# src-d/kmcuda

Measured on AMD Instinct MI355X. Metric: point-assignments/sec per Lloyd iter (8Mx256@1024), higher is better.
Workload: dtype f32

## Files before the change

kmcuda_amd/csrc/engine.cpp:

```cpp
#include "engine.hpp"

#include <math.h>
#include <stdio.h>
#include <stdlib.h>
#include <string.h>

#include <mutex>
#include <vector>

#include "../../include/kmcuda_amd.h"

namespace kmx {

int g_verbosity = 0;

namespace {
std::mutex g_stream_pool_mutex;
std::vector<std::vector<hipStream_t>> g_stream_pool;
}

hipStream_t pooled_stream_acquire(int device) {
  {
    std::lock_guard<std::mutex> lock(g_stream_pool_mutex);
    if ((size_t)device < g_stream_pool.size() && !g_stream_pool[device].empty()) {
// ... 68 lines not shown
  for (auto &s : spans_) { (void)hipEventDestroy(s.a); (void)hipEventDestroy(s.b); }
  for (void *p : owned_) (void)hipFree(p);
  if (pinned_) (void)hipHostFree(pinned_);
  if (side_stream_ && own_side_stream_) pooled_stream_release(device_, side_stream_);
  if (ev_fork_) (void)hipEventDestroy(ev_fork_);
  if (ev_join_) (void)hipEventDestroy(ev_join_);
  for (hipEvent_t e : ev_report_)
    if (e) (void)hipEventDestroy(e);
  if (ev_rows_) (void)hipEventDestroy(ev_rows_);
  if (own_stream_ && stream_) {
    if (blocking_stream_) (void)hipStreamDestroy(stream_);
    else pooled_stream_release(device_, stream_);
  }
}

int Engine::init(int device, uint32_t n_rows, uint32_t D, uint32_t K, int metric, int fp16x2, hipStream_t stream) {
  if (getenv("KMCUDA_AMD_DEBUG")) g_verbosity = atoi(getenv("KMCUDA_AMD_DEBUG"));
  if (const char *f = getenv("KMCUDA_AMD_FILTER")) filter_mode_ = strcmp(f, "f32") == 0 ? 1 : 0;
  if (const char *c = getenv("KMCUDA_AMD_ROW_CACHE")) row_cache_allowed_ = atoi(c) != 0;
  carry_pairs_ = true;
  if (const char *c = getenv("KMCUDA_AMD_CARRY_PAIRS")) carry_pairs_ = atoi(c) != 0;
  if (const char *c = getenv("KMCUDA_AMD_SETTLE")) settle_ = atoi(c) != 0;
  if (const char *c = getenv("KMCUDA_AMD_DUO")) { duo_on_ = atoi(c) != 0; duo_always_ = atoi(c) == 2; }
  if (const char *c = getenv("KMCUDA_AMD_WIDE")) wide_ok_ = atoi(c) != 0;
  if (const char *c = getenv("KMCUDA_AMD_GEMM")) wide_ok_ = atoi(c) != 0;
  if (const char *u = getenv("KMCUDA_AMD_UPDATE"))
    ms_.force = strcmp(u, "radix") == 0 ? 1 : (strcmp(u, "sync") == 0 ? 2 : (strcmp(u, "bucket") == 0 ? 3 : 0));
  if (D == 0 || K < 1 || K >= 0x7FFFFFFFu) return kInvalidArguments;
  if (fp16x2) return kInvalidArguments;
  int ndev = 0;
  if (hipGetDeviceCount(&ndev) != hipSuccess || device < 0 || device >= ndev) return kNoSuchDevice;
  KMX_HIP(hipSetDevice(device), kNoSuchDevice);
  device_ = device;
  if (stream == (hipStream_t)(intptr_t)-1) {
    KMX_HIP(hipStreamCreateWithFlags(&stream_, hipStreamDefault), kRuntimeError);
    own_stream_ = true;
    blocking_stream_ = true;
  } else if (stream) {
    stream_ = stream;
  } else {
    stream_ = pooled_stream_acquire(device);
    if (!stream_) return kRuntimeError;
    own_stream_ = true;
  }
  N_ = n_rows; D_ = D; K_ = K; metric_ = metric; fp16x2_ = fp16x2;
  K_pad_ = (K + 31) / 32 * 32;
// ... 341 lines not shown
    KMX_HIP(launch_centroid_rows(metric_, centroids, K_, D_, Kt_, csqr_, ct_, side_stream_), kRuntimeError);
    KMX_HIP(hipEventRecord(ev_rows_, side_stream_), kRuntimeError);
    rows_on_side = true;
    if (!prepared) {
      uint32_t *next = stats_;
      stats_ = stats_ == stats_base_ ? stats_base_ + 8 : stats_base_;
      KMX_HIP(launch_centroid_prep_frozen(metric_, centroids, K_, D_, K_pad_, DP_ ? DP_ : wide_dp_, mu_, finite_, bias_,
                                          bias2_, cfil_, panelhi_, stats_, next, counters_ + 1, counters_ + 3, counters_ + 4,
                                          carry_on_ ? drift_ : nullptr, carry_on_ && drift_ ? counters_ + kCarryCursor : nullptr,
                                          stream_),
              kRuntimeError);
      carry_preps_++;
    }
  } else {
    int rc = prepare_centroids(centroids);
    if (rc) return rc;
  }
  LloydArgs a;
  a.samples = samples; a.N = N_; a.D = D_; a.K = K_; a.K_pad = K_pad_; a.DP = DP_; a.Kt = Kt_;
  a.cfil = cfil_; a.bias = bias_; a.mu = mu_; a.ct = ct_; a.csqr = csqr_; a.stats = stats_;
  a.eps = eps_; a.tie_slack = tie_slack_;
  a.assignments = assignments; a.assignments_prev = assignments_prev;
  a.flagged = flagged_; a.pairs = pairs_; a.counters = counters_;
  if (N_ == 0) return kSuccess;
  if (wide_sel) {
    const int rc = lloyd_assign_wide(a, centroids, wide_steady, rows_on_side, carry_was_valid);
    if (rc != kNoSuchDevice + 100) return rc;
  }
  if (exact_only || DP_ == 0 || (DP_ > 256 && filter_mode_ != 0)) {
    span_begin(1);
    const uint32_t grid = N_ < 8192u ? N_ : 8192u;
    KMX_HIP(launch_lloyd_exact(metric_, a, nullptr, nullptr, grid, stream_), kRuntimeError);
    span_end();
    return kSuccess;
  }
  span_begin(0);
  if (two_stage) {
    const void *rows = half_rows_ ? half_rows_ : (const void *)samples;
    const bool half = half_rows_ != nullptr;
    bool duo_listed = false;
    if (!steady)
      KMX_HIP(launch_centroid_panelhi(centroids, K_, D_, K_pad_, DP_, finite_, mu_, bias_, panelhi_, stats_, stream_),
              kRuntimeError);
    if (build_cache) {
      const size_t npad = ((size_t)N_ + 255) / 256 * 256;
      if (!xcache_) {
// ... 615 lines not shown
```

kmcuda_amd/csrc/engine.hpp:

```cpp
#pragma once
#include <hip/hip_runtime.h>
#include <stdint.h>

#include <vector>

#include "kernels.hpp"

namespace kmx {

enum Result {
  kSuccess = 0, kInvalidArguments, kNoSuchDevice, kMemoryAllocationFailure, kRuntimeError, kMemoryCopyError
};

#define KMX_HIP(call, ret)                                                                   \
  do {                                                                                       \
    hipError_t e__ = (call);                                                                 \
    if (e__ != hipSuccess) {                                                                 \
      if (kmx::g_verbosity > 0)                                                              \
        printf("%s:%d -> %s (%s)\n", __FILE__, __LINE__, hipGetErrorString(e__), #call);     \
      return ret;                                                                            \
    }                                                                                        \
  } while (0)

extern int g_verbosity;
// ... 90 lines not shown

  int device_ = -1;
  hipStream_t stream_ = nullptr;
  bool own_stream_ = false, blocking_stream_ = false;
  hipStream_t side_stream_ = nullptr;
  bool own_side_stream_ = false;
  hipEvent_t ev_fork_ = nullptr, ev_join_ = nullptr;
  hipEvent_t ev_rows_ = nullptr;
  uint32_t N_ = 0, D_ = 0, K_ = 0, K_pad_ = 0, Kt_ = 0, DP_ = 0;
  int metric_ = 0, fp16x2_ = 0;
  bool strict_h2_ = false;
  float *h2_sq_ = nullptr;
  float eps_ = 0, tie_slack_ = 0;

  float *csqr_ = nullptr, *bias_ = nullptr, *bias2_ = nullptr, *cfil_ = nullptr, *ct_ = nullptr, *mu_ = nullptr;
  uint32_t *finite_ = nullptr;
  const void *half_rows_ = nullptr;
  void *panelhi_ = nullptr;
  uint32_t *undecided_ = nullptr;
  float *und_thr_ = nullptr;
  uint32_t *duo_ = nullptr;
  bool duo_on_ = true;
  bool duo_always_ = false;
  int filter_mode_ = 0;
  bool settle_ = true;
  uint32_t wide_dp_ = 0;
  bool wide_ok_ = true;
  bool wide_failed_ = false;
  void *wide_rows16_ = nullptr;
  float *wide_meta_ = nullptr;
  uint32_t *wide_cont_ = nullptr;
  int lloyd_assign_wide(const LloydArgs &a, const float *centroids, bool steady, bool rows_on_side, bool carry_was_valid);
  bool row_cache_allowed_ = true;
  bool row_cache_on_ = false, row_cache_valid_ = false, mu_frozen_ = false;
  void *xcache_ = nullptr;
  float *xmeta_ = nullptr;
  bool carry_on_ = false;
  bool carry_valid_ = false;
  uint32_t carry_preps_ = 0;
  uint32_t carry_seq_ = 0;
  CarryPolicy carry_policy_;
  float *ub_ = nullptr, *lb_ = nullptr, *drift_ = nullptr;
  bool carry_pairs_ = true;
  float *l3_ = nullptr;
  uint32_t *p1_ = nullptr, *p2_ = nullptr;
  uint32_t *carry_list_ = nullptr;
// ... 53 lines not shown
```

kmcuda_amd/csrc/kernels.hpp:

```cpp
#pragma once
#include <hip/hip_runtime.h>
#include <stdint.h>

namespace kmx {

struct LloydArgs {
  const float *samples;
  uint32_t N, D, K;
  uint32_t K_pad;
  uint32_t DP;
  uint32_t Kt;
  const float *cfil;
  const float *bias;
  const float *mu;
  const float *ct;
  const float *csqr;
  const uint32_t *stats;
  float eps;
  float tie_slack;
  uint32_t *assignments, *assignments_prev;
  uint32_t *flagged;
  uint32_t *pairs;
  uint32_t *counters;
};
constexpr uint32_t kWaveRowGridMax = 1u << 20;
inline uint32_t wave_row_grid(uint32_t n_rows) {
  const uint32_t g = (n_rows + 3u) / 4u;
  return g < kWaveRowGridMax ? (g ? g : 1u) : kWaveRowGridMax;
}
constexpr uint32_t kStopFlag = 8;
constexpr uint32_t kCarryCursor = 9, kCarrySkipped = 10;
constexpr uint32_t kCarryPaired = 12;
constexpr uint32_t kDuoCount = 14;
struct CarryArgs {
  float *ub = nullptr, *lb = nullptr;
  const uint32_t *row_list = nullptr;
  const uint32_t *n_list = nullptr;
  uint32_t *host_report = nullptr;
  uint32_t seq = 0;
  int angular = 0;
  float *l3 = nullptr;
  uint32_t *p1 = nullptr, *p2 = nullptr;
};
struct StopCtl {
  float threshold = -1.f;
  uint32_t *counters = nullptr;
// ... 295 lines not shown
```

kmcuda_amd/csrc/lloyd_carry.hip:

```cpp
#include <cstdlib>

#include "lloyd_coarse.hpp"
#include "lloyd_refine.hpp"

namespace kmx {

constexpr int kSkipRowsPerThread = 8, kSkipBlock = 256;
template <bool WIDE>
__global__ __launch_bounds__(kSkipBlock) void carry_skip_kernel(
    uint32_t N, uint32_t K, const uint32_t *__restrict__ assignments, uint32_t *__restrict__ assignments_prev,
    CarryArgs cy, const float2 *__restrict__ xmeta, const float *__restrict__ drift, const uint32_t *__restrict__ stats,
    float tie_slack, uint32_t *__restrict__ row_list, const uint32_t *__restrict__ finite, uint32_t *__restrict__ pairs,
    uint32_t *__restrict__ counters, int probe, float terms) {
  if (counters[kStopFlag] != 0u) return;
  float *__restrict__ ub = cy.ub, *__restrict__ lb = cy.lb, *__restrict__ l3 = cy.l3;
  const int angular = cy.angular;
  const float maxdrift = __uint_as_float(stats[6]);
  const float cmaxo = sqrtf(__uint_as_float(stats[2])) * 1.000001f;
  const float4 *__restrict__ wmeta = reinterpret_cast<const float4 *>(xmeta);
  const float mu_norm = WIDE ? wmeta[N].x : reinterpret_cast<const float *>(xmeta)[2 * (((size_t)N + 255) / 256 * 256)];
  const float u = 5.9604645e-8f;
  const float maxdb = __uint_as_float(stats[7]);
  const float cmaxc = sqrtf(__uint_as_float(stats[0])) * 1.000001f;
  const float eb = 4.0f * terms * u * mu_norm * (cmaxc + maxdrift);
// ... 114 lines not shown
                             float tie_slack, uint32_t *row_list, const uint32_t *finite, uint32_t *pairs,
                             uint32_t *counters, bool probe, hipStream_t st, uint32_t wide_dg) {
  const uint32_t chunk = kSkipBlock * kSkipRowsPerThread;
  if (wide_dg)
    hipLaunchKernelGGL(carry_skip_kernel<true>, dim3((N + chunk - 1) / chunk), dim3(kSkipBlock), 0, st, N, K, assignments,
                       assignments_prev, cy, reinterpret_cast<const float2 *>(xmeta), drift, stats, tie_slack, row_list,
                       finite, pairs, counters, probe ? 1 : 0, (float)(wide_dg + 8u));
  else
    hipLaunchKernelGGL(carry_skip_kernel<false>, dim3((N + chunk - 1) / chunk), dim3(kSkipBlock), 0, st, N, K, assignments,
                       assignments_prev, cy, reinterpret_cast<const float2 *>(xmeta), drift, stats, tie_slack, row_list,
                       finite, pairs, counters, probe ? 1 : 0, 520.0f);
  return hipGetLastError();
}

template <int DP>
static hipError_t launch_coarse_carry_dp(const LloydArgs &a, const void *rows, bool half_rows, const void *xcache,
                                         const float *xmeta, const void *panelhi, uint32_t *undecided, float *und_thr,
                                         const CarryArgs &cy, uint32_t rows_hint, uint32_t *duo, hipStream_t st) {
  constexpr int NSET = DP <= 256 ? 2 : 1;
  const size_t lds_bytes = 2 * 64 * (size_t)(DP * 2) + 512 + 64 + (size_t)DP * 4;
  const uint32_t rows_per_block = 128u * NSET;
  uint32_t grid = (a.N + rows_per_block - 1) / rows_per_block;
  const bool fast = a.D == (uint32_t)DP;
#define KMX_CARRY_LAUNCH(H, F, C, MODE, SRC)                                                                          \
  hipLaunchKernelGGL((lloyd_coarse2_kernel<DP, H, F, C, NSET, MODE>), dim3(grid), dim3(256), lds_bytes, st, SRC,      \
                     xmeta, a.N, a.D, reinterpret_cast<const float *>(panelhi), a.bias, a.mu, a.K_pad, a.K, a.stats,   \
                     a.eps, a.tie_slack, a.assignments, a.assignments_prev, undecided, und_thr, a.counters, cy, duo)
  if (!cy.row_list) {
    KMX_CARRY_LAUNCH(false, true, true, 1, xcache);
    return hipGetLastError();
  }
  if (rows_hint != 0xFFFFFFFFu) {
    const uint32_t want = rows_hint / rows_per_block + rows_hint / (4 * rows_per_block) + 64;
    if (want < grid) grid = want;
  }
  if (const char *v = getenv("KMCUDA_AMD_CARRY_GRID")) {
    const long cap = atol(v);
    if (cap > 0 && (uint32_t)cap < grid) grid = (uint32_t)cap;
  }
  if (half_rows) {
    if (fast) KMX_CARRY_LAUNCH(true, true, false, 2, rows); else KMX_CARRY_LAUNCH(true, false, false, 2, rows);
  } else {
    if (fast) KMX_CARRY_LAUNCH(false, true, false, 2, rows); else KMX_CARRY_LAUNCH(false, false, false, 2, rows);
  }
#undef KMX_CARRY_LAUNCH
  return hipGetLastError();
}

hipError_t launch_lloyd_coarse_carry(const LloydArgs &a, const void *rows, bool half_rows, const void *xcache,
                                     const float *xmeta, const void *panelhi, uint32_t *undecided, float *und_thr,
                                     const CarryArgs &cy, uint32_t rows_hint, uint32_t *duo, hipStream_t st) {
  switch (a.DP) {
#define KMX_CARRY_CASE(dp) \
    case dp: return launch_coarse_carry_dp<dp>(a, rows, half_rows, xcache, xmeta, panelhi, undecided, und_thr, cy, rows_hint, duo, st)
    KMX_CARRY_CASE(16); KMX_CARRY_CASE(32); KMX_CARRY_CASE(64); KMX_CARRY_CASE(128); KMX_CARRY_CASE(256); KMX_CARRY_CASE(512);
#undef KMX_CARRY_CASE
    default: return hipErrorInvalidValue;
  }
}

hipError_t launch_lloyd_refine_carry(const LloydArgs &a, const void *rows, bool half_rows, const void *panelhi,
                                     const uint32_t *row_list, const float *thr_list, const uint32_t *n_list,
                                     uint32_t rows_hint, const CarryArgs &cy, hipStream_t st) {
  return launch_lloyd_refine_t<true>(a, rows, half_rows, panelhi, row_list, thr_list, n_list, rows_hint, cy, st);
}

hipError_t preload_lloyd_carry_code() {
  hipFuncAttributes at;
// ... 5 lines not shown
```

kmcuda_amd/csrc/lloyd_coarse.hpp:

```cpp
#pragma once
#include <hip/hip_fp16.h>

#include "exact.hpp"
#include "filter_common.hpp"
#include "kernels.hpp"

#ifndef KMX_ABL
#define KMX_ABL 0
#endif

namespace kmx {

typedef float f32x16 __attribute__((ext_vector_type(16)));
typedef float f32x4 __attribute__((ext_vector_type(4)));
typedef _Float16 f16x8 __attribute__((ext_vector_type(8)));

template <int P>
struct TileParity { static constexpr int value = P; };
__device__ __forceinline__ f16x8 lds_frag_issue(uint32_t addr) {
  f16x8 f;
  asm volatile("ds_read_b128 %0, %1" : "=v"(f) : "v"(addr) : "memory");
  return f;
}
template <int N>
__device__ __forceinline__ void lds_frag_wait(f16x8 &f) {
  asm volatile("s_waitcnt lgkmcnt(%1)" : "+v"(f) : "n"(N));
}

template <int DP, bool HALF_ROWS, bool FAST, bool CACHED, int NSET, int CARRY = 0>
__global__ __launch_bounds__(256, 2) void lloyd_coarse2_kernel(
    const void *__restrict__ rows, const float *__restrict__ xmeta, uint32_t N, uint32_t D, const float *__restrict__ panelhi,
    const float *__restrict__ bias, const float *__restrict__ mu, uint32_t K_pad, uint32_t K,
    const uint32_t *__restrict__ stats, float eps, float tie_slack, uint32_t *__restrict__ assignments,
    uint32_t *__restrict__ assignments_prev, uint32_t *__restrict__ undecided, float *__restrict__ und_thr,
    uint32_t *__restrict__ counters, CarryArgs cy, uint32_t *__restrict__ duo = nullptr) {
  static_assert(CARRY == 0 || CARRY == 1 || CARRY == 2, "CARRY");
  static_assert(CARRY != 2 || !CACHED, "listed rows are gathered from the rows, not streamed from the row cache");
  constexpr int NKH = DP / 2;
  constexpr int KS = NKH / 8;
  constexpr int ROWB = DP * 2;
  constexpr int SUPB = 64 * ROWB;
  constexpr int NP = SUPB / 1024;
  constexpr int SWM = (KS < 16 ? KS : 16) - 1;
  typedef __attribute__((address_space(3))) unsigned char lds_byte;
  extern __shared__ __attribute__((aligned(1024))) unsigned char lds2[];
  if (counters[kStopFlag] != 0u) return;
  const uint32_t lds0 = (uint32_t)(uintptr_t)(lds_byte *)lds2;
  if (lds0 & 1023u) __builtin_trap();
  const uint32_t bias0 = lds0 + 2 * SUPB;
  constexpr uint32_t BIASB = 512u;

  const int tid = threadIdx.x, lane = tid & 63, wave = __builtin_amdgcn_readfirstlane(tid >> 6), col = lane & 31, h = lane >> 5;
  constexpr int WV = 4;
  constexpr bool TWO = NSET == 2;
  uint32_t total = N;
  if constexpr (CARRY == 2) total = __builtin_amdgcn_readfirstlane(*cy.n_list);
  if constexpr (CARRY != 0) {
    if (blockIdx.x == 0 && threadIdx.x == 0) {
      if (cy.host_report) {
        volatile uint32_t *hr = cy.host_report;
// ... 107 lines not shown
    const uint32_t P = (uint32_t)p * 1024u + P0;
    const uint32_t from = P ^ (((P / ROWB) & SWM) << 4);
    __builtin_amdgcn_global_load_lds((const __attribute__((address_space(1))) void *)(src + from),
                                     (__attribute__((address_space(3))) void *)(uintptr_t)(lds0 + buf * SUPB + p * 1024), 16, 0, 0);
  };
  const uint32_t mybias = bias0;
  auto stage_bias = [&](uint32_t sp, int buf) {
    __builtin_amdgcn_global_load_lds((const __attribute__((address_space(1))) void *)(biashi + sp * 64u + lane),
                                     (__attribute__((address_space(3))) void *)(uintptr_t)(mybias + buf * 256), 4, 0, 0);
  };
  auto stage_issue = [&](uint32_t sp, int buf, int nw, int me) {
    for (int p = me; p < NP; p += nw) stage_piece(sp, buf, p);
    if (me == 0) stage_bias(sp, buf);
  };

  {
    constexpr int MUP = (DP * 4 + 1023) / 1024;
    if (wave < MUP && lane * 16 < DP * 4 - wave * 1024)
      __builtin_amdgcn_global_load_lds((const __attribute__((address_space(1))) void *)(reinterpret_cast<const unsigned char *>(mu) + wave * 1024 + lane * 16),
                                       (__attribute__((address_space(3))) void *)(uintptr_t)(mu_lds + wave * 1024), 16, 0, 0);
  }
  stage_issue(0, 0, WV, wave);
  load_rows();

  float v1a[2] = {-INFINITY, -INFINITY}, v2a[2] = {-INFINITY, -INFINITY}, v1b[2] = {-INFINITY, -INFINITY}, v2b[2] = {-INFINITY, -INFINITY};
  uint32_t tba[2] = {0, 0}, tbb[2] = {0, 0};
  const uint32_t fragbase = lds0 + (uint32_t)col * ROWB + (uint32_t)h * (KS * 16) + (uint32_t)((col & SWM) * 16);
  float pinf = INFINITY;
  asm volatile("" : "+s"(pinf));
  auto pack = [&](float v, int r) { return __uint_as_float((__float_as_uint(v) & 0xFFFFFFF0u) | (uint32_t)r); };
  auto book2 = [&](float a, float b, int r, float &v1, float &v2) {
    const float pa = pack(a, r), pb = pack(b, r + 1);
    const float m = __builtin_amdgcn_fmed3f(v1, pa, pb);
    v2 = __builtin_amdgcn_fmed3f(v2, m, pinf);
    float t;
    asm("v_max3_f32 %0, %1, %2, %3" : "=v"(t) : "v"(v1), "v"(pa), "v"(pb));
    v1 = t;
  };
  auto lds_f4 = [](uint32_t addr) {
    return *reinterpret_cast<const __attribute__((address_space(3))) f32x4 *>((uintptr_t)addr);
  };
  auto load_bias = [&](uint32_t biasaddr, f32x16 &b) {
#pragma unroll
    for (int g = 0; g < 4; g++) {
      const f32x4 b4 = lds_f4(biasaddr + (8 * g + 4 * h) * 4);
      b[4 * g + 0] = b4.x; b[4 * g + 1] = b4.y; b[4 * g + 2] = b4.z; b[4 * g + 3] = b4.w;
    }
  };
  auto tile_pass = [&](uint32_t ldsbase, uint32_t biasaddr, uint32_t t, bool stage, uint32_t sp_next, int buf_next, auto parity) {
    constexpr int PAR = decltype(parity)::value;
    f32x16 accA, accB;
    load_bias(biasaddr, accA);
    accB = accA;
    uint32_t fb = fragbase + ldsbase;
    asm volatile("" : "+v"(fb));
    constexpr int PD = KS <= 3 ? KS - 1 : 3;
    f16x8 fr[PD + 1];
#pragma unroll
    for (int j = 0; j < PD; j++) fr[j] = lds_frag_issue(fb ^ (uint32_t)(j * 16));
#pragma unroll
    for (int j = 0; j < KS; j++) {
      if (j + PD < KS) fr[(j + PD) % (PD + 1)] = lds_frag_issue(fb ^ (uint32_t)((j + PD) * 16));
      constexpr int kMaxBehind = PD;
      const int behind = (KS - 1 - j) < kMaxBehind ? (KS - 1 - j) : kMaxBehind;
      f16x8 &f = fr[j % (PD + 1)];
      if (behind == 7) lds_frag_wait<7>(f);
      else if (behind == 6) lds_frag_wait<6>(f);
      else if (behind == 5) lds_frag_wait<5>(f);
      else if (behind == 4) lds_frag_wait<4>(f);
      else if (behind == 3) lds_frag_wait<3>(f);
      else if (behind == 2) lds_frag_wait<2>(f);
      else if (behind == 1) lds_frag_wait<1>(f);
      else lds_frag_wait<0>(f);
      accA = __builtin_amdgcn_mfma_f32_32x32x16_f16(f, xa[j], accA, 0, 0, 0);
      if constexpr (TWO) accB = __builtin_amdgcn_mfma_f32_32x32x16_f16(f, xb[j], accB, 0, 0, 0);
      constexpr int SPREAD = KS >= 8 ? KS / 8 : 1;
      if (!(KMX_ABL & 1) && stage && (j % SPREAD) == SPREAD / 2 && j / SPREAD < 8) {
        const int slot = j / SPREAD;
        for (int p = slot * 4 + wave; p < NP; p += 32) stage_piece(sp_next, buf_next, p);
        if (slot == 0 && wave == 0) stage_bias(sp_next, buf_next);
      }
    }
    const float v1a_in = v1a[PAR], v1b_in = v1b[PAR];
    if (KMX_ABL & 4) {
      v1a[PAR] = fmaxf(v1a[PAR], accA[0]); v2a[PAR] = fmaxf(v2a[PAR], accA[15]);
      if constexpr (TWO) { v1b[PAR] = fmaxf(v1b[PAR], accB[0]); v2b[PAR] = fmaxf(v2b[PAR], accB[15]); }
    } else {
#pragma unroll
      for (int r = 0; r < 16; r += 2) {
        book2(accA[r], accA[r + 1], r, v1a[PAR], v2a[PAR]);
        if constexpr (TWO) book2(accB[r], accB[r + 1], r, v1b[PAR], v2b[PAR]);
      }
    }
    tba[PAR] = (v1a[PAR] != v1a_in) ? t : tba[PAR];
    tbb[PAR] = (v1b[PAR] != v1b_in) ? t : tbb[PAR];
  };

  for (uint32_t sp = 0; sp < nsuper; sp++) {
    const int buf = sp & 1;
    const bool stage = sp + 1 < nsuper;
    const uint32_t base = buf * SUPB, bb = mybias + buf * 256;
    tile_pass(base, bb, 2 * sp, stage, sp + 1, buf ^ 1, TileParity<0>());
    tile_pass(base + 32 * ROWB, bb + 128, 2 * sp + 1, false, sp + 1, buf ^ 1, TileParity<1>());
    asm volatile("s_waitcnt vmcnt(0)" ::: "memory");
    if (!(KMX_ABL & 16)) __syncthreads();
  }
  if (KMX_ABL & 8) {
    if (v1a[0] + v2a[0] + v1b[0] + v2b[0] + v1a[1] + v2a[1] + v1b[1] + v2b[1] == 1.2345f) assignments[0] = tba[0] + tbb[0] + tba[1] + tbb[1];
    return;
  }

  const float cmaxc = sqrtf(__uint_as_float(stats[0])) * 1.000001f;
  const float bmaxc = __uint_as_float(stats[1]);
  const float cmaxo = sqrtf(__uint_as_float(stats[2])) * 1.000001f;
  const float mu_norm = (CACHED || CARRY == 2) ? xmeta[2 * (((size_t)N + 255) / 256 * 256)] : cmaxo;
  const float dcmax = sqrtf(__uint_as_float(stats[5])) * 1.000001f;
  const float u = 5.9604645e-8f;
  uint32_t und_count = 0, changed_count = 0, duo_count = 0;
  unsigned long long uma = 0, umb = 0, dma = 0, dmb = 0;
  bool unda = false, undb = false, duoa = false, duob = false;
  uint32_t d1a = 0, d2a = 0, d1b = 0, d2b = 0;
  float dra = 0.f, drb = 0.f;
  const bool want_duo = duo != nullptr;
  const bool angular = tie_slack > 0.f;
  auto finish = [&](uint32_t s, bool live, const float (&q1)[2], const float (&q2)[2], const uint32_t (&qt)[2], float xn2,
                    float x0, float dx2, float xdm, float xab, bool &und, unsigned long long &um, float &cut, bool &is_duo,
                    unsigned long long &dm, uint32_t &dc1, uint32_t &dc2, float &drest) {
    const bool insane = (x0 != x0);
    auto index_of = [&](float v, uint32_t tb, uint32_t hh) {
      const uint32_t r = __float_as_uint(v) & 15u;
      return tb * 32u + (r & 3u) + 8u * (r >> 2) + 4u * hh;
    };
    float k0 = q1[0], k1 = q1[1], k2 = __shfl_xor(q1[0], 32), k3 = __shfl_xor(q1[1], 32);
    uint32_t j0 = index_of(k0, qt[0], h), j1 = index_of(k1, qt[1], h);
    uint32_t j2 = __shfl_xor(j0, 32), j3 = __shfl_xor(j1, 32);
    const float mine2 = fmaxf(q2[0], q2[1]);
    const float others = fmaxf(mine2, __shfl_xor(mine2, 32));
    auto order = [](float &a, uint32_t &ia, float &b, uint32_t &ib) {
      const bool g = b > a;
      const float ta = g ? b : a, tb2 = g ? a : b;
      const uint32_t ja = g ? ib : ia, jb = g ? ia : ib;
      a = ta; b = tb2; ia = ja; ib = jb;
    };
    order(k0, j0, k1, j1); order(k2, j2, k3, j3); order(k0, j0, k2, j2); order(k1, j1, k3, j3); order(k1, j1, k2, j2);
    float v1 = k0;
    const uint32_t i1 = j0;
    const float v2 = fmaxf(k1, others);
    const float xn = sqrtf(xn2) * 1.0001f, xo = (xn + mu_norm) * 1.0001f;
    const float dx = dx2 >= 0.f ? sqrtf(dx2) * 1.0001f : 4.8829e-4f * xn;
    const float e_c = 2.0f * eps * (xn * cmaxc + bmaxc) + (xn * dcmax + dx * cmaxc + dx * dcmax) * 1.001f +
                      6e-8f * sqrtf((float)DP) * (xn + cmaxc) + 2.0e-6f * (1.001f * xn * cmaxc + bmaxc);
    const float e_ref = u * (12.0f * xo * cmaxo + 4.0f * cmaxo * cmaxo);
    const float thr = 2.0f * (e_c + e_ref) * 1.001f + tie_slack;
    const bool in_range = (xn < 6.0e4f) && (cmaxc < 6.0e4f) && (v1 > -1.0e38f) && (i1 < K);
    const ClampLimits lim = clamp_limits(angular, xdm, dot_error(DP, xab >= 0.f ? xab : xo * mu_norm), 0.5f * thr);
    const bool certain = insane || (in_range && ((v1 - v2) > thr) && (v2 < lim.hi) && (v1 > lim.lo));
    const bool mine = (h == 0) && live;
    bool changed = false;
    if (mine && certain) changed = commit_row(s, insane ? K : i1, assignments, assignments_prev);
    und = mine && !certain;
    is_duo = false;
    {
      float c0 = in_range ? v1 - thr : __builtin_nanf("");
      if (angular) c0 = (lim.hi == lim.hi) ? fminf(c0, lim.hi) : __builtin_nanf("");
      is_duo = want_duo && und && (k1 >= c0) && (k2 < c0) && (others < c0) && (j1 < K);
      if (is_duo) und = false;
      dc1 = j0; dc2 = j1; drest = fmaxf(k2, others);
    }
    if constexpr (CARRY != 0) {
      if (mine && cy.angular) {
        const float e = e_c * 1.001f;
        float gapv = (certain && !insane && in_range)
                         ? fminf(fminf((v1 - e) - (v2 + e), lim.hi - v2), v1 - lim.lo) * 0.999999f : -INFINITY;
        if (!(gapv == gapv)) gapv = -INFINITY;
        cy.ub[s] = gapv;
        if (cy.l3) cy.l3[s] = 0.f;
      } else if (mine) {
        float ubv = INFINITY, lbv = 0.f;
        if (!insane && in_range) {
          const float e = e_c * 1.001f;
// ... 25 lines not shown
    xn2a = ma.x; dx2a = ma.y; xn2b = mb.x; dx2b = mb.y;
    x0a = (ma.y == -1.f) ? __builtin_nanf("") : 0.f;
    x0b = (mb.y == -1.f) ? __builtin_nanf("") : 0.f;
    xaba = xabb = -1.f;
    if (angular) {
      const float *xdot = xmeta + 2 * (((size_t)N + 255) / 256 * 256) + 2;
      xdma = xdot[sA];
      xdmb = xdot[TWO ? sB : sA];
    }
  } else if (angular) {
    const uint32_t fb = (uint32_t)(h * NKH), fe = min(fb + (uint32_t)NKH, D);
    if (fb < fe) {
      if constexpr (HALF_ROWS) {
        row_dot_mu(reinterpret_cast<const _Float16 *>(rows) + (size_t)(liveA ? sA : 0u) * D, mu, fb, fe, xdma, xaba);
        if constexpr (TWO) row_dot_mu(reinterpret_cast<const _Float16 *>(rows) + (size_t)(liveB ? sB : 0u) * D, mu, fb, fe, xdmb, xabb);
      } else {
        row_dot_mu(reinterpret_cast<const float *>(rows) + (size_t)(liveA ? sA : 0u) * D, mu, fb, fe, xdma, xaba);
        if constexpr (TWO) row_dot_mu(reinterpret_cast<const float *>(rows) + (size_t)(liveB ? sB : 0u) * D, mu, fb, fe, xdmb, xabb);
      }
    }
    xdma += __shfl_xor(xdma, 32); xaba += __shfl_xor(xaba, 32);
    xdmb += __shfl_xor(xdmb, 32); xabb += __shfl_xor(xabb, 32);
  }
  float cuta, cutb;
  finish(sA, liveA, v1a, v2a, tba, xn2a, x0a, dx2a, xdma, xaba, unda, uma, cuta, duoa, dma, d1a, d2a, dra);
  cutb = 0.f;
  if constexpr (TWO) finish(sB, liveB, v1b, v2b, tbb, xn2b, x0b, dx2b, xdmb, xabb, undb, umb, cutb, duob, dmb, d1b, d2b, drb);
  __shared__ uint32_t blk_und[WV], blk_changed[WV], blk_duo[WV], blk_base, blk_duo_base;
  if (lane == 0) {
    blk_und[wave] = und_count;
    blk_changed[wave] = changed_count;
    blk_duo[wave] = duo_count;
  }
  __syncthreads();
  if (threadIdx.x == 0) {
    uint32_t tu = 0, tc = 0, td = 0;
#pragma unroll
    for (int w = 0; w < WV; w++) {
      tu += blk_und[w];
      tc += blk_changed[w];
      td += blk_duo[w];
    }
    if (tc) atomicAdd(&counters[0], tc);
    blk_base = tu ? atomicAdd(&counters[4], tu) : 0u;
    blk_duo_base = td ? atomicAdd(&counters[kDuoCount], td) : 0u;
  }
  __syncthreads();
  if (duo_count) {
    uint32_t base = blk_duo_base;
    for (int w = 0; w < wave; w++) base += blk_duo[w];
// ... 37 lines not shown
```

kmcuda_amd/csrc/lloyd_f16.hip:

```cpp
#include <hip/hip_fp16.h>

#include "exact.hpp"
#include "filter_common.hpp"
#include "kernels.hpp"
#include "lloyd_coarse.hpp"
#include "lloyd_refine.hpp"

namespace kmx {

__global__ __launch_bounds__(256) void centroid_panelhi_kernel(
    const float *__restrict__ centroids, uint32_t K, uint32_t D, uint32_t K_pad, uint32_t DP,
    const uint32_t *__restrict__ finite, const float *__restrict__ mu, const float *__restrict__ bias,
    _Float16 *__restrict__ panelhi, uint32_t K_pad64, uint32_t *__restrict__ stats) {
  const uint32_t lane = threadIdx.x & 63, wave = threadIdx.x >> 6;
  const uint32_t c = blockIdx.x * 4 + wave;
  uint32_t res_bits = 0;
  if (c < K_pad64) {
    const bool real = c < K_pad;
    const bool ok = c < K && finite[c];
    float res2 = 0.f;
    for (uint32_t f = lane; f < DP; f += 64) {
      float v = 0.f;
      if (ok && f < D) v = centroids[(size_t)c * D + f] - mu[f];
      const _Float16 hi = (_Float16)v;
// ... 177 lines not shown
}


hipError_t launch_centroid_panelhi(const float *centroids, uint32_t K, uint32_t D, uint32_t K_pad, uint32_t DP,
                                   const uint32_t *finite, const float *mu, const float *bias, void *panelhi,
                                   uint32_t *stats, hipStream_t st) {
  const uint32_t K_pad64 = (K_pad + 63u) / 64u * 64u;
  hipLaunchKernelGGL(centroid_panelhi_kernel, dim3(K_pad64 / 4), dim3(256), 0, st, centroids, K, D, K_pad, DP, finite,
                     mu, bias, reinterpret_cast<_Float16 *>(panelhi), K_pad64, stats);
  return hipGetLastError();
}

bool lloyd_filter_f16_supported(uint32_t D, uint32_t DP) { return DP >= 16 && D <= DP; }

template <int DP>
static hipError_t launch_coarse2_dp(const LloydArgs &a, const void *rows, bool half_rows, const void *xcache,
                                    const float *xmeta, const void *panelhi, uint32_t *undecided, float *und_thr,
                                    uint32_t *duo, hipStream_t st) {
  constexpr int NSET = DP <= 256 ? 2 : 1;
  const size_t lds_bytes = 2 * 64 * (size_t)(DP * 2) + 512 + 64 + (size_t)DP * 4;
  const uint32_t rows_per_block = 128u * NSET;
  const uint32_t grid = (a.N + rows_per_block - 1) / rows_per_block;
  const bool fast = a.D == (uint32_t)DP;
#define KMX_CRS2_LAUNCH(H, F, C, SRC)                                                                              \
  hipLaunchKernelGGL((lloyd_coarse2_kernel<DP, H, F, C, NSET>), dim3(grid), dim3(256), lds_bytes, st, SRC, xmeta,   \
                     a.N, a.D, reinterpret_cast<const float *>(panelhi), a.bias, a.mu, a.K_pad, a.K, a.stats,       \
                     a.eps, a.tie_slack, a.assignments, a.assignments_prev, undecided, und_thr, a.counters, CarryArgs(), duo)
  if (xcache) {
    KMX_CRS2_LAUNCH(false, true, true, xcache);
  } else if (half_rows) {
    if (fast) KMX_CRS2_LAUNCH(true, true, false, rows); else KMX_CRS2_LAUNCH(true, false, false, rows);
  } else {
    if (fast) KMX_CRS2_LAUNCH(false, true, false, rows); else KMX_CRS2_LAUNCH(false, false, false, rows);
  }
#undef KMX_CRS2_LAUNCH
  return hipGetLastError();
}

hipError_t launch_lloyd_coarse(const LloydArgs &a, const void *rows, bool half_rows, const void *xcache,
                               const float *xmeta, const void *panelhi, uint32_t *undecided, float *und_thr,
                               uint32_t *duo, hipStream_t st) {
  switch (a.DP) {
    case 16: return launch_coarse2_dp<16>(a, rows, half_rows, xcache, xmeta, panelhi, undecided, und_thr, duo, st);
    case 32: return launch_coarse2_dp<32>(a, rows, half_rows, xcache, xmeta, panelhi, undecided, und_thr, duo, st);
    case 64: return launch_coarse2_dp<64>(a, rows, half_rows, xcache, xmeta, panelhi, undecided, und_thr, duo, st);
    case 128: return launch_coarse2_dp<128>(a, rows, half_rows, xcache, xmeta, panelhi, undecided, und_thr, duo, st);
    case 256: return launch_coarse2_dp<256>(a, rows, half_rows, xcache, xmeta, panelhi, undecided, und_thr, duo, st);
    case 512: return launch_coarse2_dp<512>(a, rows, half_rows, xcache, xmeta, panelhi, undecided, und_thr, duo, st);
    default: return hipErrorInvalidValue;
  }
}

hipError_t launch_lloyd_refine(const LloydArgs &a, const void *rows, bool half_rows, const void *panelhi,
                               const uint32_t *row_list, const float *thr_list, const uint32_t *n_list,
                               uint32_t rows_hint, hipStream_t st) {
  return launch_lloyd_refine_t<false>(a, rows, half_rows, panelhi, row_list, thr_list, n_list, rows_hint, CarryArgs(), st);
}

// ... 101 lines not shown
```

Baseline: 2.078 billion.

## Add 16x16x32 MFMA variant of coarse assignment kernel, default on

Adds a SHAPE template parameter to the coarse filter kernel. When there are two row sets and DP>=32, the kernel now uses 16x16x32 f16 MFMA instead of 32x32x16. Row fragments are rearranged with permlane16 swaps, a new fragment addressing and swizzle is used, and the top-2 reduction across lane groups is rewritten to match. This is meant to cut MFMA latency and register pressure, and to improve how instruction issue interleaves with the LDS fragment reads. It adds a new index-decoding path that must match the 16x16 output layout exactly. The 32-wide shape can be selected back through an environment variable.

Result: faster. 2.201 billion (median of 6 runs) (+5.9%).

```diff
diff --git a/kmcuda_amd/csrc/engine.cpp b/kmcuda_amd/csrc/engine.cpp
--- a/kmcuda_amd/csrc/engine.cpp
+++ b/kmcuda_amd/csrc/engine.cpp
@@ -114,6 +114,7 @@
   if (const char *c = getenv("KMCUDA_AMD_CARRY_PAIRS")) carry_pairs_ = atoi(c) != 0;
   if (const char *c = getenv("KMCUDA_AMD_SETTLE")) settle_ = atoi(c) != 0;
   if (const char *c = getenv("KMCUDA_AMD_DUO")) { duo_on_ = atoi(c) != 0; duo_always_ = atoi(c) == 2; }
+  if (const char *c = getenv("KMCUDA_AMD_COARSE_MFMA")) coarse_mfma_ = atoi(c) == 32 ? 32u : 16u;
   if (const char *c = getenv("KMCUDA_AMD_WIDE")) wide_ok_ = atoi(c) != 0;
   if (const char *c = getenv("KMCUDA_AMD_GEMM")) wide_ok_ = atoi(c) != 0;
   if (const char *u = getenv("KMCUDA_AMD_UPDATE"))
@@ -501,6 +502,7 @@
   a.eps = eps_; a.tie_slack = tie_slack_;
   a.assignments = assignments; a.assignments_prev = assignments_prev;
   a.flagged = flagged_; a.pairs = pairs_; a.counters = counters_;
+  a.coarse_mfma = coarse_mfma_;
   if (N_ == 0) return kSuccess;
   if (wide_sel) {
     const int rc = lloyd_assign_wide(a, centroids, wide_steady, rows_on_side, carry_was_valid);
diff --git a/kmcuda_amd/csrc/engine.hpp b/kmcuda_amd/csrc/engine.hpp
--- a/kmcuda_amd/csrc/engine.hpp
+++ b/kmcuda_amd/csrc/engine.hpp
@@ -136,6 +136,7 @@
   uint32_t *duo_ = nullptr;
   bool duo_on_ = true;
   bool duo_always_ = false;
+  uint32_t coarse_mfma_ = 16;
   int filter_mode_ = 0;
   bool settle_ = true;
   uint32_t wide_dp_ = 0;
diff --git a/kmcuda_amd/csrc/kernels.hpp b/kmcuda_amd/csrc/kernels.hpp
--- a/kmcuda_amd/csrc/kernels.hpp
+++ b/kmcuda_amd/csrc/kernels.hpp
@@ -22,6 +22,7 @@
   uint32_t *flagged;
   uint32_t *pairs;
   uint32_t *counters;
+  uint32_t coarse_mfma = 16;
 };
 constexpr uint32_t kWaveRowGridMax = 1u << 20;
 inline uint32_t wave_row_grid(uint32_t n_rows) {
diff --git a/kmcuda_amd/csrc/lloyd_carry.hip b/kmcuda_amd/csrc/lloyd_carry.hip
--- a/kmcuda_amd/csrc/lloyd_carry.hip
+++ b/kmcuda_amd/csrc/lloyd_carry.hip
@@ -160,10 +160,17 @@
   const uint32_t rows_per_block = 128u * NSET;
   uint32_t grid = (a.N + rows_per_block - 1) / rows_per_block;
   const bool fast = a.D == (uint32_t)DP;
-#define KMX_CARRY_LAUNCH(H, F, C, MODE, SRC)                                                                          \
-  hipLaunchKernelGGL((lloyd_coarse2_kernel<DP, H, F, C, NSET, MODE>), dim3(grid), dim3(256), lds_bytes, st, SRC,      \
-                     xmeta, a.N, a.D, reinterpret_cast<const float *>(panelhi), a.bias, a.mu, a.K_pad, a.K, a.stats,   \
+  constexpr bool kS16 = NSET == 2 && DP >= 32;
+  const bool s16 = kS16 && a.coarse_mfma != 32;
+#define KMX_CARRY_LAUNCH_S(H, F, C, MODE, SRC, SHAPE)                                                                       \
+  hipLaunchKernelGGL((lloyd_coarse2_kernel<DP, H, F, C, NSET, MODE, SHAPE>), dim3(grid), dim3(256), lds_bytes, st, SRC,     \
+                     xmeta, a.N, a.D, reinterpret_cast<const float *>(panelhi), a.bias, a.mu, a.K_pad, a.K, a.stats,        \
                      a.eps, a.tie_slack, a.assignments, a.assignments_prev, undecided, und_thr, a.counters, cy, duo)
+#define KMX_CARRY_LAUNCH(H, F, C, MODE, SRC)                           \
+  do {                                                                 \
+    if (s16) KMX_CARRY_LAUNCH_S(H, F, C, MODE, SRC, (kS16 && !(MODE == 2 && DP >= 256)) ? 16 : 32); \
+    else KMX_CARRY_LAUNCH_S(H, F, C, MODE, SRC, 32);                   \
+  } while (0)
   if (!cy.row_list) {
     KMX_CARRY_LAUNCH(false, true, true, 1, xcache);
     return hipGetLastError();
@@ -182,6 +189,7 @@
     if (fast) KMX_CARRY_LAUNCH(false, true, false, 2, rows); else KMX_CARRY_LAUNCH(false, false, false, 2, rows);
   }
 #undef KMX_CARRY_LAUNCH
+#undef KMX_CARRY_LAUNCH_S
   return hipGetLastError();
 }
 
diff --git a/kmcuda_amd/csrc/lloyd_coarse.hpp b/kmcuda_amd/csrc/lloyd_coarse.hpp
--- a/kmcuda_amd/csrc/lloyd_coarse.hpp
+++ b/kmcuda_amd/csrc/lloyd_coarse.hpp
@@ -22,12 +22,30 @@
   asm volatile("ds_read_b128 %0, %1" : "=v"(f) : "v"(addr) : "memory");
   return f;
 }
+template <int OFF>
+__device__ __forceinline__ f16x8 lds_frag_issue_off(uint32_t addr) {
+  f16x8 f;
+  asm volatile("ds_read_b128 %0, %1 offset:%2" : "=v"(f) : "v"(addr), "n"(OFF) : "memory");
+  return f;
+}
 template <int N>
 __device__ __forceinline__ void lds_frag_wait(f16x8 &f) {
   asm volatile("s_waitcnt lgkmcnt(%1)" : "+v"(f) : "n"(N));
 }
-
-template <int DP, bool HALF_ROWS, bool FAST, bool CACHED, int NSET, int CARRY = 0>
+__device__ __forceinline__ void frag_swap16(f16x8 &p, f16x8 &q) {
+  typedef uint32_t u32x4 __attribute__((ext_vector_type(4)));
+  u32x4 a = __builtin_bit_cast(u32x4, p), b = __builtin_bit_cast(u32x4, q);
+#pragma unroll
+  for (int d = 0; d < 4; d++) {
+    const auto r = __builtin_amdgcn_permlane16_swap(a[d], b[d], false, false);
+    a[d] = r[0];
+    b[d] = r[1];
+  }
+  p = __builtin_bit_cast(f16x8, a);
+  q = __builtin_bit_cast(f16x8, b);
+}
+
+template <int DP, bool HALF_ROWS, bool FAST, bool CACHED, int NSET, int CARRY = 0, int SHAPE = 32>
 __global__ __launch_bounds__(256, 2) void lloyd_coarse2_kernel(
     const void *__restrict__ rows, const float *__restrict__ xmeta, uint32_t N, uint32_t D, const float *__restrict__ panelhi,
     const float *__restrict__ bias, const float *__restrict__ mu, uint32_t K_pad, uint32_t K,
@@ -36,6 +54,8 @@
     uint32_t *__restrict__ counters, CarryArgs cy, uint32_t *__restrict__ duo = nullptr) {
   static_assert(CARRY == 0 || CARRY == 1 || CARRY == 2, "CARRY");
   static_assert(CARRY != 2 || !CACHED, "listed rows are gathered from the rows, not streamed from the row cache");
+  static_assert(SHAPE == 32 || (SHAPE == 16 && NSET == 2 && DP >= 32), "16x16x32: two row sets, 32 features per k-step");
+  constexpr bool S16 = SHAPE == 16;
   constexpr int NKH = DP / 2;
   constexpr int KS = NKH / 8;
   constexpr int ROWB = DP * 2;
@@ -189,10 +209,23 @@
   }
   stage_issue(0, 0, WV, wave);
   load_rows();
+  if constexpr (S16) {
+#pragma unroll
+    for (int p = 0; p < KS / 2; p++) {
+      frag_swap16(xa[2 * p], xa[2 * p + 1]);
+      frag_swap16(xb[2 * p], xb[2 * p + 1]);
+    }
+  }
 
   float v1a[2] = {-INFINITY, -INFINITY}, v2a[2] = {-INFINITY, -INFINITY}, v1b[2] = {-INFINITY, -INFINITY}, v2b[2] = {-INFINITY, -INFINITY};
   uint32_t tba[2] = {0, 0}, tbb[2] = {0, 0};
-  const uint32_t fragbase = lds0 + (uint32_t)col * ROWB + (uint32_t)h * (KS * 16) + (uint32_t)((col & SWM) * 16);
+  float w1[4], w2[4];
+  uint32_t wt[4];
+#pragma unroll
+  for (int q = 0; q < 4; q++) { w1[q] = w2[q] = -INFINITY; wt[q] = 0; }
+  const uint32_t fragbase =
+      S16 ? lds0 + (uint32_t)(lane & 15) * ROWB + (uint32_t)h * (KS * 16) + (uint32_t)(((((lane >> 4) & 1) ^ (lane & 15)) & SWM) * 16)
+          : lds0 + (uint32_t)col * ROWB + (uint32_t)h * (KS * 16) + (uint32_t)((col & SWM) * 16);
   float pinf = INFINITY;
   asm volatile("" : "+s"(pinf));
   auto pack = [&](float v, int r) { return __uint_as_float((__float_as_uint(v) & 0xFFFFFFF0u) | (uint32_t)r); };
@@ -214,39 +247,96 @@
       b[4 * g + 0] = b4.x; b[4 * g + 1] = b4.y; b[4 * g + 2] = b4.z; b[4 * g + 3] = b4.w;
     }
   };
+  constexpr int PD = KS <= 3 ? KS - 1 : 3;
+  auto frag_wait = [&](int j, f16x8 &f) {
+    constexpr int kMaxBehind = PD;
+    const int behind = (KS - 1 - j) < kMaxBehind ? (KS - 1 - j) : kMaxBehind;
+    if (behind == 7) lds_frag_wait<7>(f);
+    else if (behind == 6) lds_frag_wait<6>(f);
+    else if (behind == 5) lds_frag_wait<5>(f);
+    else if (behind == 4) lds_frag_wait<4>(f);
+    else if (behind == 3) lds_frag_wait<3>(f);
+    else if (behind == 2) lds_frag_wait<2>(f);
+    else if (behind == 1) lds_frag_wait<1>(f);
+    else lds_frag_wait<0>(f);
+  };
+  auto stage_after = [&](int j, bool stage, uint32_t sp_next, int buf_next) {
+    constexpr int SPREAD = KS >= 8 ? KS / 8 : 1;
+    if (!(KMX_ABL & 1) && stage && (j % SPREAD) == SPREAD / 2 && j / SPREAD < 8) {
+      const int slot = j / SPREAD;
+      for (int p = slot * 4 + wave; p < NP; p += 32) stage_piece(sp_next, buf_next, p);
+      if (slot == 0 && wave == 0) stage_bias(sp_next, buf_next);
+    }
+  };
+  auto tile_pass16 = [&](uint32_t ldsbase, uint32_t biasaddr, uint32_t t, bool stage, uint32_t sp_next, int buf_next) {
+    const int g = lane >> 4;
+    f32x4 acc[2][4];
+#pragma unroll
+    for (int b = 0; b < 2; b++) {
+      const f32x4 b4 = lds_f4(biasaddr + (16 * b + 4 * g) * 4);
+#pragma unroll
+      for (int q = 0; q < 4; q++) acc[b][q] = b4;
+    }
+    uint32_t fb = fragbase + ldsbase;
+    asm volatile("" : "+v"(fb));
+    auto issue = [&](int j) {
+      const uint32_t a = fb ^ (uint32_t)((j >> 1) * 32);
+      return (j & 1) ? lds_frag_issue_off<16 * ROWB>(a) : lds_frag_issue(a);
+    };
+    f16x8 fr[PD + 1];
+#pragma unroll
+    for (int j = 0; j < PD; j++) fr[j] = issue(j);
+#pragma unroll
+    for (int j = 0; j < KS; j++) {
+      if (j + PD < KS) fr[(j + PD) % (PD + 1)] = issue(j + PD);
+      f16x8 &f = fr[j % (PD + 1)];
+      frag_wait(j, f);
+      const int b = j & 1, p = j >> 1;
+      acc[b][0] = __builtin_amdgcn_mfma_f32_16x16x32_f16(f, xa[2 * p], acc[b][0], 0, 0, 0);
+      acc[b][1] = __builtin_amdgcn_mfma_f32_16x16x32_f16(f, xa[2 * p + 1], acc[b][1], 0, 0, 0);
+      acc[b][2] = __builtin_amdgcn_mfma_f32_16x16x32_f16(f, xb[2 * p], acc[b][2], 0, 0, 0);
+      acc[b][3] = __builtin_amdgcn_mfma_f32_16x16x32_f16(f, xb[2 * p + 1], acc[b][3], 0, 0, 0);
+      stage_after(j, stage, sp_next, buf_next);
+    }
+    float w1_in[4];
+#pragma unroll
+    for (int q = 0; q < 4; q++) w1_in[q] = w1[q];
+    if (KMX_ABL & 4) {
+#pragma unroll
+      for (int q = 0; q < 4; q++) { w1[q] = fmaxf(w1[q], acc[0][q][0]); w2[q] = fmaxf(w2[q], acc[1][q][3]); }
+    } else {
+#pragma unroll
+      for (int b = 0; b < 2; b++)
+#pragma unroll
+        for (int i = 0; i < 4; i += 2)
+#pragma unroll
+          for (int q = 0; q < 4; q++) book2(acc[b][q][i], acc[b][q][i + 1], 4 * b + i, w1[q], w2[q]);
+    }
+#pragma unroll
+    for (int q = 0; q < 4; q++) wt[q] = (w1[q] != w1_in[q]) ? t : wt[q];
+  };
   auto tile_pass = [&](uint32_t ldsbase, uint32_t biasaddr, uint32_t t, bool stage, uint32_t sp_next, int buf_next, auto parity) {
     constexpr int PAR = decltype(parity)::value;
+    if constexpr (S16) {
+      tile_pass16(ldsbase, biasaddr, t, stage, sp_next, buf_next);
+      return;
+    }
     f32x16 accA, accB;
     load_bias(biasaddr, accA);
     accB = accA;
     uint32_t fb = fragbase + ldsbase;
     asm volatile("" : "+v"(fb));
-    constexpr int PD = KS <= 3 ? KS - 1 : 3;
     f16x8 fr[PD + 1];
 #pragma unroll
     for (int j = 0; j < PD; j++) fr[j] = lds_frag_issue(fb ^ (uint32_t)(j * 16));
 #pragma unroll
     for (int j = 0; j < KS; j++) {
       if (j + PD < KS) fr[(j + PD) % (PD + 1)] = lds_frag_issue(fb ^ (uint32_t)((j + PD) * 16));
-      constexpr int kMaxBehind = PD;
-      const int behind = (KS - 1 - j) < kMaxBehind ? (KS - 1 - j) : kMaxBehind;
       f16x8 &f = fr[j % (PD + 1)];
-      if (behind == 7) lds_frag_wait<7>(f);
-      else if (behind == 6) lds_frag_wait<6>(f);
-      else if (behind == 5) lds_frag_wait<5>(f);
-      else if (behind == 4) lds_frag_wait<4>(f);
-      else if (behind == 3) lds_frag_wait<3>(f);
-      else if (behind == 2) lds_frag_wait<2>(f);
-      else if (behind == 1) lds_frag_wait<1>(f);
-      else lds_frag_wait<0>(f);
+      frag_wait(j, f);
       accA = __builtin_amdgcn_mfma_f32_32x32x16_f16(f, xa[j], accA, 0, 0, 0);
       if constexpr (TWO) accB = __builtin_amdgcn_mfma_f32_32x32x16_f16(f, xb[j], accB, 0, 0, 0);
-      constexpr int SPREAD = KS >= 8 ? KS / 8 : 1;
-      if (!(KMX_ABL & 1) && stage && (j % SPREAD) == SPREAD / 2 && j / SPREAD < 8) {
-        const int slot = j / SPREAD;
-        for (int p = slot * 4 + wave; p < NP; p += 32) stage_piece(sp_next, buf_next, p);
-        if (slot == 0 && wave == 0) stage_bias(sp_next, buf_next);
-      }
+      stage_after(j, stage, sp_next, buf_next);
     }
     const float v1a_in = v1a[PAR], v1b_in = v1b[PAR];
     if (KMX_ABL & 4) {
@@ -273,7 +363,11 @@
     if (!(KMX_ABL & 16)) __syncthreads();
   }
   if (KMX_ABL & 8) {
-    if (v1a[0] + v2a[0] + v1b[0] + v2b[0] + v1a[1] + v2a[1] + v1b[1] + v2b[1] == 1.2345f) assignments[0] = tba[0] + tbb[0] + tba[1] + tbb[1];
+    float keep = 0.f;
+    uint32_t keept = 0;
+#pragma unroll
+    for (int q = 0; q < (S16 ? 4 : 1); q++) { keep += w1[q] + w2[q]; keept += wt[q]; }
+    if (v1a[0] + v2a[0] + v1b[0] + v2b[0] + v1a[1] + v2a[1] + v1b[1] + v2b[1] + keep == 1.2345f) assignments[0] = tba[0] + tbb[0] + tba[1] + tbb[1] + keept;
     return;
   }
 
@@ -290,19 +384,44 @@
   float dra = 0.f, drb = 0.f;
   const bool want_duo = duo != nullptr;
   const bool angular = tie_slack > 0.f;
-  auto finish = [&](uint32_t s, bool live, const float (&q1)[2], const float (&q2)[2], const uint32_t (&qt)[2], float xn2,
-                    float x0, float dx2, float xdm, float xab, bool &und, unsigned long long &um, float &cut, bool &is_duo,
-                    unsigned long long &dm, uint32_t &dc1, uint32_t &dc2, float &drest) {
-    const bool insane = (x0 != x0);
+  auto quarters32 = [&](const float (&q1)[2], const float (&q2)[2], const uint32_t (&qt)[2], float (&kq)[4],
+                        uint32_t (&jq)[4], float &others) {
     auto index_of = [&](float v, uint32_t tb, uint32_t hh) {
       const uint32_t r = __float_as_uint(v) & 15u;
       return tb * 32u + (r & 3u) + 8u * (r >> 2) + 4u * hh;
     };
-    float k0 = q1[0], k1 = q1[1], k2 = __shfl_xor(q1[0], 32), k3 = __shfl_xor(q1[1], 32);
-    uint32_t j0 = index_of(k0, qt[0], h), j1 = index_of(k1, qt[1], h);
-    uint32_t j2 = __shfl_xor(j0, 32), j3 = __shfl_xor(j1, 32);
+    kq[0] = q1[0]; kq[1] = q1[1]; kq[2] = __shfl_xor(q1[0], 32); kq[3] = __shfl_xor(q1[1], 32);
+    jq[0] = index_of(kq[0], qt[0], h); jq[1] = index_of(kq[1], qt[1], h);
+    jq[2] = __shfl_xor(jq[0], 32); jq[3] = __shfl_xor(jq[1], 32);
     const float mine2 = fmaxf(q2[0], q2[1]);
-    const float others = fmaxf(mine2, __shfl_xor(mine2, 32));
+    others = fmaxf(mine2, __shfl_xor(mine2, 32));
+  };
+  auto quarters16 = [&](float (&kq)[4], uint32_t (&jq)[4], float &others) {
+    const int g = lane >> 4;
+    float o[4];
+#pragma unroll
+    for (int r = 0; r < 4; r++) {
+      const int gq = g ^ r;
+      auto pick = [&](const auto (&a)[4]) {
+        const auto lo = (gq & 1) ? a[1] : a[0], hi = (gq & 1) ? a[3] : a[2];
+        return (gq & 2) ? hi : lo;
+      };
+      float v = pick(w1), v2 = pick(w2);
+      uint32_t tb = pick(wt);
+      if (r) { v = __shfl_xor(v, 16 * r); v2 = __shfl_xor(v2, 16 * r); tb = __shfl_xor(tb, 16 * r); }
+      const uint32_t ri = __float_as_uint(v) & 15u;
+      kq[r] = v;
+      o[r] = v2;
+      jq[r] = tb * 32u + 16u * (ri >> 2) + 4u * (uint32_t)gq + (ri & 3u);
+    }
+    others = fmaxf(fmaxf(o[0], o[1]), fmaxf(o[2], o[3]));
+  };
+  auto finish = [&](uint32_t s, bool mine, const float (&kq)[4], const uint32_t (&jq)[4], float others, float xn2,
+                    float x0, float dx2, float xdm, float xab, bool &und, unsigned long long &um, float &cut, bool &is_duo,
+                    unsigned long long &dm, uint32_t &dc1, uint32_t &dc2, float &drest) {
+    const bool insane = (x0 != x0);
+    float k0 = kq[0], k1 = kq[1], k2 = kq[2], k3 = kq[3];
+    uint32_t j0 = jq[0], j1 = jq[1], j2 = jq[2], j3 = jq[3];
     auto order = [](float &a, uint32_t &ia, float &b, uint32_t &ib) {
       const bool g = b > a;
       const float ta = g ? b : a, tb2 = g ? a : b;
@@ -322,7 +441,6 @@
     const bool in_range = (xn < 6.0e4f) && (cmaxc < 6.0e4f) && (v1 > -1.0e38f) && (i1 < K);
     const ClampLimits lim = clamp_limits(angular, xdm, dot_error(DP, xab >= 0.f ? xab : xo * mu_norm), 0.5f * thr);
     const bool certain = insane || (in_range && ((v1 - v2) > thr) && (v2 < lim.hi) && (v1 > lim.lo));
-    const bool mine = (h == 0) && live;
     bool changed = false;
     if (mine && certain) changed = commit_row(s, insane ? K : i1, assignments, assignments_prev);
     und = mine && !certain;
@@ -394,10 +512,23 @@
     xdma += __shfl_xor(xdma, 32); xaba += __shfl_xor(xaba, 32);
     xdmb += __shfl_xor(xdmb, 32); xabb += __shfl_xor(xabb, 32);
   }
-  float cuta, cutb;
-  finish(sA, liveA, v1a, v2a, tba, xn2a, x0a, dx2a, xdma, xaba, unda, uma, cuta, duoa, dma, d1a, d2a, dra);
-  cutb = 0.f;
-  if constexpr (TWO) finish(sB, liveB, v1b, v2b, tbb, xn2b, x0b, dx2b, xdmb, xabb, undb, umb, cutb, duob, dmb, d1b, d2b, drb);
+  float cuta, cutb = 0.f;
+  float kq[4], oth;
+  uint32_t jq[4];
+  if constexpr (S16) {
+    quarters16(kq, jq, oth);
+    const bool mine = h ? liveB : liveA;
+    sA = h ? sB : sA;
+    finish(sA, mine, kq, jq, oth, h ? xn2b : xn2a, h ? x0b : x0a, h ? dx2b : dx2a, h ? xdmb : xdma, h ? xabb : xaba, unda, uma,
+           cuta, duoa, dma, d1a, d2a, dra);
+  } else {
+    quarters32(v1a, v2a, tba, kq, jq, oth);
+    finish(sA, h == 0 && liveA, kq, jq, oth, xn2a, x0a, dx2a, xdma, xaba, unda, uma, cuta, duoa, dma, d1a, d2a, dra);
+    if constexpr (TWO) {
+      quarters32(v1b, v2b, tbb, kq, jq, oth);
+      finish(sB, h == 0 && liveB, kq, jq, oth, xn2b, x0b, dx2b, xdmb, xabb, undb, umb, cutb, duob, dmb, d1b, d2b, drb);
+    }
+  }
   __shared__ uint32_t blk_und[WV], blk_changed[WV], blk_duo[WV], blk_base, blk_duo_base;
   if (lane == 0) {
     blk_und[wave] = und_count;
diff --git a/kmcuda_amd/csrc/lloyd_f16.hip b/kmcuda_amd/csrc/lloyd_f16.hip
--- a/kmcuda_amd/csrc/lloyd_f16.hip
+++ b/kmcuda_amd/csrc/lloyd_f16.hip
@@ -223,10 +223,17 @@
   const uint32_t rows_per_block = 128u * NSET;
   const uint32_t grid = (a.N + rows_per_block - 1) / rows_per_block;
   const bool fast = a.D == (uint32_t)DP;
-#define KMX_CRS2_LAUNCH(H, F, C, SRC)                                                                              \
-  hipLaunchKernelGGL((lloyd_coarse2_kernel<DP, H, F, C, NSET>), dim3(grid), dim3(256), lds_bytes, st, SRC, xmeta,   \
-                     a.N, a.D, reinterpret_cast<const float *>(panelhi), a.bias, a.mu, a.K_pad, a.K, a.stats,       \
+  constexpr bool kS16 = NSET == 2 && DP >= 32;
+  const bool s16 = kS16 && a.coarse_mfma != 32;
+#define KMX_CRS2_LAUNCH_S(H, F, C, SRC, SHAPE)                                                                            \
+  hipLaunchKernelGGL((lloyd_coarse2_kernel<DP, H, F, C, NSET, 0, SHAPE>), dim3(grid), dim3(256), lds_bytes, st, SRC, xmeta, \
+                     a.N, a.D, reinterpret_cast<const float *>(panelhi), a.bias, a.mu, a.K_pad, a.K, a.stats,             \
                      a.eps, a.tie_slack, a.assignments, a.assignments_prev, undecided, und_thr, a.counters, CarryArgs(), duo)
+#define KMX_CRS2_LAUNCH(H, F, C, SRC)                       \
+  do {                                                      \
+    if (s16) KMX_CRS2_LAUNCH_S(H, F, C, SRC, kS16 ? 16 : 32); \
+    else KMX_CRS2_LAUNCH_S(H, F, C, SRC, 32);               \
+  } while (0)
   if (xcache) {
     KMX_CRS2_LAUNCH(false, true, true, xcache);
   } else if (half_rows) {
@@ -235,6 +242,7 @@
     if (fast) KMX_CRS2_LAUNCH(false, true, false, rows); else KMX_CRS2_LAUNCH(false, false, false, rows);
   }
 #undef KMX_CRS2_LAUNCH
+#undef KMX_CRS2_LAUNCH_S
   return hipGetLastError();
 }
 
```
